# teboli/polyblur

Measured on AMD Instinct MI355X. Metric: megapixels/sec (n_iter=3, alpha=6, beta=1), higher is better.
Workload: dtype f32; 1 GPU; batch=1 3840x2160x3 fp32 per GPU, n_iter=3, method=fft (circular), full 25-tap support; mode=resident, images_per_gpu=1, height=2160, width=3840, parallelism=images sharded, no data-path collective

## Files before the change

polyblur_amd/build.py:

```python
from __future__ import annotations

import hashlib
import os
import shutil
import subprocess
import sys
from concurrent.futures import ThreadPoolExecutor

HERE = os.path.dirname(os.path.abspath(__file__))
CSRC = os.path.join(HERE, "csrc")
LIBDIR = os.path.join(HERE, "lib")
LIBNAME = "libpolyblur_hip.so"
SOURCES = ["api.hip", "comm.hip", "conv.hip", "conv_fft.hip", "conv_big.hip", "conv_wfft.hip", "conv_w128.hip", "estimate.hip", "lines_fixed.hip", "filters.hip", "nc.hip"]
EXPERIMENTAL_SOURCES = ["conv_strip.hip", "conv_xt.hip"]
ARCH = "gfx950"
FLAGS = ["-O3", "-std=c++17", "-fPIC", "--offload-arch=" + ARCH, "-Wall", "-Wno-unused-function"]


def hipcc_path() -> str:
    for cand in (os.environ.get("HIPCC"), shutil.which("hipcc"), "/opt/rocm/bin/hipcc"):
        if cand and os.path.exists(cand):
            return cand
    raise RuntimeError("hipcc not found (set HIPCC or install ROCm)")


def lib_path() -> str:
    return os.path.join(LIBDIR, LIBNAME)


def _newer(target: str, deps) -> bool:
    if not os.path.exists(target):
        return True
    t = os.path.getmtime(target)
    return any(os.path.getmtime(d) > t for d in deps)


def build(force: bool = False, verbose: bool = True, experimental: bool = False) -> str:
    os.makedirs(LIBDIR, exist_ok=True)
    hipcc = hipcc_path()
    headers = [os.path.join(CSRC, f) for f in os.listdir(CSRC) if f.endswith(".h")]
    headers.append(os.path.join(os.path.dirname(HERE), "include", "polyblur_hip.h"))
    jobs = []
    objs = []
    extra = os.environ.get("PB_EXTRA_FLAGS", "").split()
    flags = FLAGS + extra
    sources = SOURCES + (EXPERIMENTAL_SOURCES if experimental else [])
    if experimental:
        flags = flags + ["-DPB_EXPERIMENTAL"]
    flavour = hashlib.sha256(" ".join(flags + sources).encode()).hexdigest()[:10]
    objdir = os.path.join(LIBDIR, "obj" if not (extra or experimental) else "obj-" + flavour)
    os.makedirs(objdir, exist_ok=True)
    stamp = os.path.join(LIBDIR, "flavour.txt")
    relink = not os.path.exists(stamp) or open(stamp).read().strip() != flavour
    for src in sources:
        s = os.path.join(CSRC, src)
        o = os.path.join(objdir, src.replace(".hip", ".o"))
        objs.append(o)
        if force or _newer(o, [s] + headers):
            jobs.append([hipcc] + flags + ["-c", s, "-o", o])

    def run(cmd):
        if verbose:
            print(" ".join(cmd), flush=True)
        r = subprocess.run(cmd, capture_output=True, text=True)
        if r.returncode != 0:
            raise RuntimeError("hipcc failed:\n%s\n%s" % (r.stdout, r.stderr))
        if verbose and r.stderr.strip():
            print(r.stderr, file=sys.stderr)

    with ThreadPoolExecutor(max_workers=4) as ex:
        list(ex.map(run, jobs))
    out = lib_path()
    if jobs or relink or not os.path.exists(out):
        run([hipcc, "-shared", "-fPIC", "--offload-arch=" + ARCH, "-o", out] + objs + ["-ldl"])
        with open(stamp, "w") as f:
            f.write(flavour + "\n")
    return out


if __name__ == "__main__":
    print(build(force="--force" in sys.argv, experimental="--experimental" in sys.argv))
```

polyblur_amd/csrc/api.hip:

```cpp
#include <cstdlib>
#include <cstring>

#include "common.h"

int pb_grad_energy(pb_ctx *ctx, const void *gx, const void *gy, float *nM, int P, long HW, int g_dtype = PB_F32);
int pb_halo_apply(pb_ctx *ctx, const void *x, int x_dtype, int x_pitch, long x_plane, const float *y, const void *gx,
                  const void *gy, const void *ox, const float *nM, void *out, int out_dtype, int P, int H, int W,
                  int clamp01, const void *recomb_cur = nullptr, int recomb_cur_dtype = 0, const float *recomb_smooth = nullptr,
                  int g_dtype = PB_F32);
int pb_recombine(pb_ctx *ctx, const float *y, const void *cur, int cur_dtype, const float *smooth, void *out, int out_dtype,
                 long n);
int pb_bilateral5_impl(pb_ctx *ctx, const void *in, int in_dtype, void *out, int out_dtype, int P, int H, int W);
int pb_dt_filter_impl(pb_ctx *ctx, const void *in, const void *joint, int dtype, float *out, int B, int C, int H, int W,
                      float sigma_s, float sigma_r, int num_iterations);
int pb_nc_filter_impl(pb_ctx *ctx, const void *in, int dtype, float *out, int B, int C, int H, int W, float sigma_s,
                      float sigma_r, int num_iterations);
int pb_convert_from_float(pb_ctx *ctx, const float *in, void *out, int dtype, long n);
int pb_u8_layout(pb_ctx *ctx, const unsigned char *in, unsigned char *out, int B, int C, int H, int W, int to_planar);
int pb_convert_to_float(pb_ctx *ctx, const void *in, int dtype, float *out, long n);
int pb_extract_patches_impl(pb_ctx *ctx, const void *img, void *patches, int dtype, int B, int C, int H, int W, int ph, int pw,
                            int step_h, int step_w, int n_j, int pad_top, int pad_left, int first, int count);
int pb_overlap_add_impl(pb_ctx *ctx, const void *patches, void *out, int dtype, int B, int C, int H, int W, int ph, int pw,
                        int step_h, int step_w, int n_i, int n_j, int pad_top, int pad_left, const float *win_y,
                        const float *win_x);
// ... 23 lines not shown
    }
    const size_t want = (bytes + 255) & ~(size_t)255;
    if (hipMalloc(&b.p, want) != hipSuccess) {
        b.p = nullptr;
        pb_fail(ctx, PB_ERR_NOMEM, "scratch '%s': hipMalloc(%zu) failed", name, want);
        return nullptr;
    }
    b.bytes = want;
    return b.p;
}

static size_t dsize(int dtype) { return dtype == PB_F16 ? 2 : (dtype == PB_U8 ? 1 : 4); }
static int pitch4(int w) { return (w + 3) & ~3; }

static void pb_read_knobs(pb_ctx *ctx) {
    auto geti = [](const char *n, int &v) { if (const char *e = getenv(n)) v = atoi(e); };
    auto getl = [](const char *n, long &v) { if (const char *e = getenv(n)) v = atol(e); };
    if (const char *e = getenv("PB_FFT_BODY")) ctx->fft_wave = (e[0] == 'w' && e[1] == 'g') ? 0 : 1;
#ifdef PB_EXPERIMENTAL
    geti("PB_STRIP", ctx->strip_mode);
#endif
    geti("PB_EST_GRAY_ROWS", ctx->est_gray_rows); geti("PB_EST_LEAN", ctx->est_lean); geti("PB_DT_ROWS_REG", ctx->dt_rows_reg); geti("PB_DT_COLS_STRIP", ctx->dt_cols_strip); geti("PB_DT_COLS_COOP", ctx->dt_cols_coop);
    geti("PB_FFT_EXT_RADIX", ctx->fft_ext_radix); geti("PB_FFT_FIRST", ctx->fft_first); geti("PB_FFT_FIRST_ROWS", ctx->fft_first_rows); geti("PB_COLS_FIXED", ctx->cols_fixed); geti("PB_ROWS_FIXED", ctx->rows_fixed);
    geti("PB_POLY1", ctx->poly_mode);
    geti("PB_POLY_ALWAYS", ctx->poly_always); geti("PB_POLY_PADDED", ctx->poly_padded); geti("PB_TAPER_RING", ctx->taper_ring); geti("PB_ZERO_RING", ctx->zero_ring); getl("PB_ZERO_RING_MIN_PAIRS", ctx->zero_ring_min_pairs);
}

extern "C" {

int pb_version(void) { return PB_VERSION; }

void pb_default_options(pb_options *o) {
    memset(o, 0, sizeof(*o));
    o->n_iter = 1; o->c = 0.352f; o->b = 0.768f; o->alpha = 2.f; o->beta = 3.f;
    o->sigma_r = 0.8f; o->sigma_s = 2.0f; o->q = 0.f; o->n_angles = 6; o->n_interpolated_angles = 30;
    o->remove_halo = 0; o->edgetaping = 0; o->prefilter = PB_PREFILTER_NONE; o->discard_saturation = 0;
    o->boundary = PB_WRAP; o->support = PB_SUPPORT_FULL; o->force_theta_deg = -1.f; o->ker_size = PB_KSIZE;
}

int pb_create(pb_ctx **out, int device, void *stream) {
    if (!out) return PB_ERR_BADARG;
    *out = nullptr;
    int n = 0;
    if (hipGetDeviceCount(&n) != hipSuccess || n <= 0 || device < 0 || device >= n) return PB_ERR_HIP;
    if (hipSetDevice(device) != hipSuccess) return PB_ERR_HIP;
    pb_ctx *ctx = new pb_ctx();
    ctx->device = device;
    ctx->stream = static_cast<hipStream_t>(stream);
    pb_read_knobs(ctx);
    if (hipEventCreate(&ctx->ev0) != hipSuccess || hipEventCreate(&ctx->ev1) != hipSuccess ||
        hipEventCreateWithFlags(&ctx->ev_switch, hipEventDisableTiming) != hipSuccess) { delete ctx; return PB_ERR_HIP; }
    {
        if (hipStreamCreateWithFlags(&ctx->aux, hipStreamNonBlocking) != hipSuccess ||
            hipEventCreateWithFlags(&ctx->ev_fork, hipEventDisableTiming) != hipSuccess ||
            hipEventCreateWithFlags(&ctx->ev_join, hipEventDisableTiming) != hipSuccess) {
            (void)hipGetLastError();
            if (ctx->aux) (void)hipStreamDestroy(ctx->aux);
            ctx->aux = nullptr;
        }
    }
    *out = ctx;
    return PB_OK;
}

int pb_set_dense_eval(pb_ctx *ctx, int mode, int min_phases) {
    if (!ctx || (mode != PB_DENSE_STENCIL && mode != PB_DENSE_AUTO) || min_phases < 0 || min_phases > PB_MAX_PHASES + 1)
        return PB_ERR_BADARG;
    ctx->fft_min_phases = mode == PB_DENSE_STENCIL ? -1 : min_phases;
    pb_forget_hints(ctx);
    return PB_OK;
}

// ... 795 lines not shown
```

polyblur_amd/csrc/common.h:

```cpp
#pragma once
#include <hip/hip_runtime.h>
#include <hip/hip_fp16.h>

#include <cstdarg>
#include <cstdio>
#include <map>
#include <string>
#include <vector>

#include "../../include/polyblur_hip.h"


struct FftPlan {
    int n = 0;
    int nstage = 0;
    int radix[24];
    int bluestein_m = 0;
    float2 *tw = nullptr;
    float *drev = nullptr;
    float2 *chirp = nullptr;
    float2 *bfilt_rev = nullptr;
    float *dnat = nullptr;
};

// ... 66 lines not shown
    int sel_slot = 0, sel_last = 0, sel_B = 0;
    const std::vector<pb_fft_sel> *known_sel = nullptr;
    SpectraSet spectra;
    int poly_mode = 3;
    PolySpec poly_want = no_poly();
    PolySpec poly_want2 = no_poly();
    SpectraSet spectra2;
    unsigned sel2_mask = 0;
    long zero_ring_min_pairs = 4096;
    int zero_ring = 1;
    int taper_ring = 1;
    int poly_padded = 1;
    int est_lean = 1;
    int dt_cols_strip = 1;
    int dt_cols_coop = 1;
    int dt_rows_reg = 1;
    int poly_always = 1;
    int est_gray_rows = 1;
    int fft_ext_radix = 1;
    int fft_first_rows = -1;
    int fft_first = -1;
    int cols_fixed = 1;
    int rows_fixed = 1;
    int strip_mode = 0;
};

int pb_fail(pb_ctx *ctx, int code, const char *fmt, ...);

struct ProfScope {
    pb_ctx *ctx;
    int idx = -1;
    ProfScope(pb_ctx *c, int tag) : ctx(c) {
        if (!c->prof_on) return;
        ProfRec r;
        r.tag = tag;
        hipEvent_t *ev[2] = {&r.a, &r.b};
        for (auto e : ev) {
            if (!c->evpool.empty()) { *e = c->evpool.back(); c->evpool.pop_back(); }
            else if (hipEventCreate(e) != hipSuccess) return;
        }
        (void)hipEventRecord(r.a, c->stream);
        c->prof.push_back(r);
        idx = (int)c->prof.size() - 1;
    }
    ~ProfScope() {
        if (idx >= 0) (void)hipEventRecord(ctx->prof[idx].b, ctx->stream);
// ... 41 lines not shown
    void *out;       int out_kind; int out_dtype; int out_pitch; long out_plane;
    int H, W;
    int pad;
    int C;
    int P;
    const pb_blur_info *info;
    float scale, coef;
    int boundary;
    int epilogue;
    int clamp01;
    int skip_sep;
    int skip_general;
    const pb_fft_sel *fsel;
    const float *khat;
    int khat_ready;
    int strip;
    int poly;
    void *out2;  int out2_kind;  int out2_pitch;  long out2_plane;  int clamp2;
    int no_fft;
    int ring;
};

int pb_launch_conv(pb_ctx *ctx, const ConvPass &p);
int pb_launch_conv_poly(pb_ctx *ctx, const ConvPass *steps);
int pb_launch_conv_xt(pb_ctx *ctx, const ConvPass &p);
int pb_build_khat(pb_ctx *ctx, const pb_blur_info *info, int B, float **khat, pb_fft_sel **sel, bool launch);
int pb_build_khat_ring(pb_ctx *ctx, const pb_blur_info *info, int B, float **khat, pb_fft_sel **sel);
int pb_khat_buffers(pb_ctx *ctx, int B, float **khat, pb_fft_sel **sel);
int pb_khat2_buffers(pb_ctx *ctx, int B, float **khat, pb_fft_sel **sel);
inline const PolySpec &pb_spec_of_spectra(const pb_ctx *ctx, const void *khat) {
    return ctx->spectra2.built_into(khat) ? ctx->spectra2.spec() : ctx->spectra.spec();
}
int pb_cache_records(pb_ctx *ctx, const pb_blur_info *info, int B);
void pb_forget_range(pb_ctx *ctx, const void *dst, size_t bytes);
inline void pb_forget_records(pb_ctx *ctx, const void *info, int B) { pb_forget_range(ctx, info, sizeof(pb_blur_info) * (size_t)B); }
void pb_forget_hints(pb_ctx *ctx);
int pb_launch_conv_fft(pb_ctx *ctx, const ConvPass &p);
int pb_launch_conv_strip(pb_ctx *ctx, const ConvPass &p);
int pb_launch_conv_wfft(pb_ctx *ctx, const ConvPass &p);
bool pb_conv_fft_types(const ConvPass &p);
bool pb_conv_wfft_types(const ConvPass &p);
int pb_launch_conv_w128(pb_ctx *ctx, const ConvPass &p);
bool pb_conv_w128_feasible(const ConvPass &p);
bool pb_conv_wfft_feasible(const ConvPass &p, bool poly2);
bool pb_conv_w128_types(int in_dtype, int out_dtype);
bool pb_poly_three_steps_ok(pb_ctx *ctx, const ConvPass *steps);
// ... 38 lines not shown
```

polyblur_amd/csrc/conv_w128.hip:

```cpp

#include <algorithm>
#include <cstdlib>
#include <type_traits>

#include "conv_wave_common.h"

namespace {

constexpr int W_N = 128;
constexpr int W_P = 129;
constexpr size_t kW128Lds = sizeof(float2) * 64 * W_P;

static __device__ const float kC128[64] = {
    1.0f, 0.9987954497337341f, 0.9951847195625305f, 0.9891765117645264f, 0.9807852506637573f, 0.9700312614440918f,
    0.9569403529167175f, 0.9415440559387207f, 0.9238795042037964f, 0.903989315032959f, 0.8819212913513184f, 0.8577286005020142f,
    0.8314695954322815f, 0.803207516670227f, 0.7730104327201843f, 0.7409511208534241f, 0.7071067690849304f, 0.6715589761734009f,
    0.6343932747840881f, 0.5956993103027344f, 0.5555702447891235f, 0.5141027569770813f, 0.4713967442512512f, 0.4275550842285156f,
    0.3826834261417389f, 0.3368898630142212f, 0.290284663438797f, 0.24298018217086792f, 0.19509032368659973f, 0.1467304676771164f,
    0.0980171412229538f, 0.049067676067352295f, 6.123234262925839e-17f, -0.049067676067352295f, -0.0980171412229538f, -0.1467304676771164f,
    -0.19509032368659973f, -0.24298018217086792f, -0.290284663438797f, -0.3368898630142212f, -0.3826834261417389f, -0.4275550842285156f,
    -0.4713967442512512f, -0.5141027569770813f, -0.5555702447891235f, -0.5956993103027344f, -0.6343932747840881f, -0.6715589761734009f,
    -0.7071067690849304f, -0.7409511208534241f, -0.7730104327201843f, -0.803207516670227f, -0.8314695954322815f, -0.8577286005020142f,
    -0.8819212913513184f, -0.903989315032959f, -0.9238795042037964f, -0.9415440559387207f, -0.9569403529167175f, -0.9700312614440918f,
    -0.9807852506637573f, -0.9891765117645264f, -0.9951847195625305f, -0.9987954497337341f};
// ... 98 lines not shown
#define PB_WT_PASS , tr
#else
#define PB_WT(i)
#define PB_WRT(i)
#define PB_WT_ARG
#define PB_WT_PASS
#endif

struct W128Geom { int ow, oh; };
struct W128Jobs { int pairs_x, njobs, per; float inv_pairs_x; };
__device__ __forceinline__ int div_rcp128(int n, float rcp_d) { return (int)(((float)n + 0.5f) * rcp_d); }
__device__ __forceinline__ W128Jobs jobs128_of(const W128Geom &g, int hx, int hy) {
    const int Tx = W_N - 2 * hx, Ty = W_N - 2 * hy;
    const int tiles_x = div_rcp128(g.ow + Tx - 1, __builtin_amdgcn_rcpf((float)Tx)), tiles_y = div_rcp128(g.oh + Ty - 1, __builtin_amdgcn_rcpf((float)Ty));
    W128Jobs j;
    j.pairs_x = (tiles_x + 1) >> 1;
    j.njobs = j.pairs_x * tiles_y;
    j.per = (j.njobs + 7) >> 3;
    j.inv_pairs_x = __builtin_amdgcn_rcpf((float)j.pairs_x);
    return j;
}

template <typename TIn, typename TOut, bool ZERO>
__device__ __forceinline__ void w128_pair(const ConvPass &a, int plane, int ty, int pxi, int hx, int hy, float2 *Z, const float *kp PB_WT_ARG) {
    constexpr int kBoundary = ZERO ? PB_ZERO : PB_WRAP;
    const int Tx = W_N - 2 * hx, Ty = W_N - 2 * hy;
    const int w = (int)(threadIdx.x >> 6), lane = (int)(threadIdx.x & 63), c = lane & 31, h = lane >> 5;
    const bool upper = h != 0;
    const float sg = upper ? -1.f : 1.f;
    const OutRegion rg = out_region(a);
    const int oy0 = rg.y_lo + ty * Ty, wy0 = oy0 - hy;
    const int wxA = rg.x_lo + 2 * pxi * Tx - hx, wxB = wxA + Tx;
    const bool hasB = wxB + hx < rg.x_hi;
    const int x = 32 * w + c;
    const TIn *ipl = static_cast<const TIn *>(a.in) + (long)plane * a.in_plane;
    TOut *opl = static_cast<TOut *>(a.out) + (long)plane * a.out_plane;
    const int Hp = a.H + 2 * a.pad, Wp = a.W + 2 * a.pad;
    cf v[64];
    PB_WT(1);

    {
        const brsrc rin = plane_rsrc(ipl, a.in_plane);
        const int lo = a.in_kind == SRC_VIRTUAL ? a.pad : 0;
        const int pitchb = a.in_pitch * (int)sizeof(TIn);
        const bool x_inside = wxA >= lo && wxB + W_N <= Wp - lo && hasB;
        const bool y_inside = wy0 >= lo && wy0 + W_N <= Hp - lo;
        const bool inside = x_inside && y_inside;
        const bool pieces = x_inside && (y_inside || Hp >= 2 * W_N) && ((a.in_pitch | (wxA - lo)) & 3) == 0;
        if (sizeof(TIn) == 4) {
            char *zw = reinterpret_cast<char *>(Z) + w * (int)(kW128Lds / 4);
// ... 204 lines not shown
            const int row0 = 64 * h;
            const int rlo = max(hy - row0, 0), rhi = min(rmax - row0, 64);
            const unsigned baseA = okA && rlo < rhi ? (unsigned)((wy0 + row0 + rlo - oo) * opitchb + (pxA - oo) * (int)sizeof(TOut)) : kNoAccess;
            const unsigned baseB = okB && rlo < rhi ? (unsigned)((wy0 + row0 + rlo - oo) * opitchb + (pxB - oo) * (int)sizeof(TOut)) : kNoAccess;
#pragma unroll
            for (int r = 0; r < 64; ++r) {
                const bool rok = r >= rlo && r < rhi;
                cf ea = v[r], eb = v[r];
                swap_halves(ea, eb);
                const cf er = ea + eb * sg;
                const float ra = __builtin_amdgcn_fmed3f(er.x, clo, chi), rb = __builtin_amdgcn_fmed3f(er.y, clo, chi);
                BufIO<TOut>::st(ro, rok ? baseA + (unsigned)((r - rlo) * opitchb) : kNoAccess, 0, ra);
                BufIO<TOut>::st(ro, rok ? baseB + (unsigned)((r - rlo) * opitchb) : kNoAccess, 0, rb);
            }
        }
    }
    PB_WT(8);
    PB_WRT(10);
}

template <typename TIn, typename TOut, bool ZERO>
__global__ __launch_bounds__(256, 2) void conv_w128_kernel(const ConvPass a, const W128Geom g) {
    extern __shared__ __attribute__((aligned(16))) float2 Zw[];
    const int lane = threadIdx.x & 63;
#if defined(PB_EXPERIMENTAL) && defined(PB_W128_TRACE)
    unsigned long long *tr = (blockIdx.x < kTraceGroups && threadIdx.x < 64) ? g_w128_trace + (long)blockIdx.x * kTraceStamps : nullptr;
    PB_WT(0);
    PB_WRT(9);
#endif
    const int C = a.C, B = a.P / C;
    const int q = (int)(blockIdx.x & 7u);
    int rem = (int)(blockIdx.x >> 3);
    int img = 0, hx = 0, hy = 0;
    if (B == 1) {
        const PB_CONSTANT pb_fft_sel *s0 = as_constant(a.fsel);
        if (!s0->use_fft || s0->poly != 2) return;
        hx = s0->hx; hy = s0->hy;
    } else {
        auto share_of = [&](int i) -> int {
            if (i >= B) return 0;
            const pb_fft_sel s = a.fsel[i];
            if (!s.use_fft || s.poly != 2) return 0;
            return jobs128_of(g, s.hx, s.hy).per * C;
        };
        bool work = false;
        int base = 0;
        for (int c0 = 0; c0 < B; c0 += 64) {
            const int n = share_of(c0 + lane), incl = wave_scan(n, lane);
            const unsigned long long m = __ballot(base + incl > rem);
            if (m) {
                const int l = __builtin_ctzll(m);
                img = c0 + l;
                rem -= base + (__builtin_amdgcn_readlane(incl, l) - __builtin_amdgcn_readlane(n, l));
                work = true;
                break;
            }
            base += __builtin_amdgcn_readlane(incl, 63);
        }
        if (!work) return;
        img = __builtin_amdgcn_readfirstlane(img); rem = __builtin_amdgcn_readfirstlane(rem);
        hx = as_constant(a.fsel + img)->hx; hy = as_constant(a.fsel + img)->hy;
    }
    const W128Jobs j = jobs128_of(g, hx, hy);
    const int pl = __builtin_amdgcn_readfirstlane(div_rcp128(rem, __builtin_amdgcn_rcpf((float)j.per)));
    if (pl >= C) return;
    const int pair = q * j.per + (rem - pl * j.per);
    if (pair >= j.njobs) return;
    const int ty = __builtin_amdgcn_readfirstlane(div_rcp128(pair, j.inv_pairs_x)), pxi = pair - ty * j.pairs_x;
    w128_pair<TIn, TOut, ZERO>(a, img * C + pl, ty, pxi, hx, hy, Zw, a.khat + (long)img * PB_KHAT_STRIDE PB_WT_PASS);
}

template <typename TIn, typename TOut>
int launch_w128_typed(pb_ctx *ctx, const ConvPass &p, const W128Geom &g, long groups) {
    if (p.boundary == PB_ZERO)
        hipLaunchKernelGGL((conv_w128_kernel<TIn, TOut, true>), dim3((unsigned)groups), dim3(256), kW128Lds, ctx->stream, p, g);
    else
        hipLaunchKernelGGL((conv_w128_kernel<TIn, TOut, false>), dim3((unsigned)groups), dim3(256), kW128Lds, ctx->stream, p, g);
    PB_LAUNCH_CHECK();
    return PB_OK;
}

}

#if defined(PB_EXPERIMENTAL) && defined(PB_W128_TRACE)
extern "C" int pb_debug_w128_trace(unsigned long long *host) {
    int rc = (int)hipMemcpyFromSymbol(host, HIP_SYMBOL(g_w128_trace), sizeof(g_w128_trace));
    static unsigned long long zeros[kTraceGroups * kTraceStamps];
    if (!rc) rc = (int)hipMemcpyToSymbol(HIP_SYMBOL(g_w128_trace), zeros, sizeof(zeros));
    return rc;
}
#endif

// ... 11 lines not shown
    W128Geom g;
    g.oh = (p.out_kind == OUT_INTERIOR) ? p.H : p.H + 2 * p.pad;
    g.ow = (p.out_kind == OUT_INTERIOR) ? p.W : p.W + 2 * p.pad;
    long groups = 0;
    const int B = p.P / p.C;
    auto per_of = [&](int hx, int hy) -> long {
        const int tx = W_N - 2 * hx, ty = W_N - 2 * hy;
        const long nj = (long)(((g.ow + tx - 1) / tx + 1) / 2) * ((g.oh + ty - 1) / ty);
        return (nj + 7) / 8;
    };
    if (ctx->known_sel) {
        long per_sum = 0;
        for (int b = 0; b < B && b < (int)ctx->known_sel->size(); ++b) {
            const pb_fft_sel &e = (*ctx->known_sel)[(size_t)b];
            if (e.use_fft && e.poly == 2) per_sum += per_of(e.hx, e.hy);
        }
        if (!per_sum) return PB_OK;
        groups = 8L * per_sum * p.C;
    } else {
        const int hmax = (W_N - PB_POLY128_MIN_T) / 2;
        groups = 8L * per_of(hmax, hmax) * p.P;
    }
    if (groups <= 0 || groups > (1L << 23)) return pb_fail(ctx, PB_ERR_UNSUPPORTED, "conv pass: too many 128 x 128 windows");
    ProfScope prof(ctx, PB_PROF_CONV_FFT);
    switch (p.in_dtype * 3 + p.out_dtype) {
        case 0: return launch_w128_typed<float, float>(ctx, p, g, groups);
        case 1: return launch_w128_typed<float, __half>(ctx, p, g, groups);
        case 3: return launch_w128_typed<__half, float>(ctx, p, g, groups);
        case 4: return launch_w128_typed<__half, __half>(ctx, p, g, groups);
        case 2: return launch_w128_typed<float, unsigned char>(ctx, p, g, groups);
        case 5: return launch_w128_typed<__half, unsigned char>(ctx, p, g, groups);
        case 6: return launch_w128_typed<unsigned char, float>(ctx, p, g, groups);
        case 7: return launch_w128_typed<unsigned char, __half>(ctx, p, g, groups);
        case 8: return launch_w128_typed<unsigned char, unsigned char>(ctx, p, g, groups);
        default: return PB_ERR_UNSUPPORTED;
    }
}
```

polyblur_amd/csrc/conv_wave_common.h:

```cpp
#pragma once
#include "conv_fft_common.h"

namespace {

constexpr int WF_ROWS = 32;
constexpr size_t kWfLdsWave = sizeof(float2) * WF_ROWS * FT_P;

static __device__ const float kC64[64] = {
    1.0f, 0.9951847195625305f, 0.9807852506637573f, 0.9569403529167175f, 0.9238795042037964f, 0.8819212913513184f,
    0.8314695954322815f, 0.7730104327201843f, 0.7071067690849304f, 0.6343932747840881f, 0.5555702447891235f,
    0.4713967442512512f, 0.3826834261417389f, 0.290284663438797f, 0.19509032368659973f, 0.0980171412229538f, 0.0f,
    -0.0980171412229538f, -0.19509032368659973f, -0.290284663438797f, -0.3826834261417389f, -0.4713967442512512f,
    -0.5555702447891235f, -0.6343932747840881f, -0.7071067690849304f, -0.7730104327201843f, -0.8314695954322815f,
    -0.8819212913513184f, -0.9238795042037964f, -0.9569403529167175f, -0.9807852506637573f, -0.9951847195625305f, -1.0f,
    -0.9951847195625305f, -0.9807852506637573f, -0.9569403529167175f, -0.9238795042037964f, -0.8819212913513184f,
    -0.8314695954322815f, -0.7730104327201843f, -0.7071067690849304f, -0.6343932747840881f, -0.5555702447891235f,
    -0.4713967442512512f, -0.3826834261417389f, -0.290284663438797f, -0.19509032368659973f, -0.0980171412229538f, 0.0f,
    0.0980171412229538f, 0.19509032368659973f, 0.290284663438797f, 0.3826834261417389f, 0.4713967442512512f,
    0.5555702447891235f, 0.6343932747840881f, 0.7071067690849304f, 0.7730104327201843f, 0.8314695954322815f,
    0.8819212913513184f, 0.9238795042037964f, 0.9569403529167175f, 0.9807852506637573f, 0.9951847195625305f};
static __device__ const float kS64[64] = {
    0.0f, 0.0980171412229538f, 0.19509032368659973f, 0.290284663438797f, 0.3826834261417389f, 0.4713967442512512f,
    0.5555702447891235f, 0.6343932747840881f, 0.7071067690849304f, 0.7730104327201843f, 0.8314695954322815f,
    0.8819212913513184f, 0.9238795042037964f, 0.9569403529167175f, 0.9807852506637573f, 0.9951847195625305f, 1.0f,
// ... 111 lines not shown

__device__ __forceinline__ int wave_scan(int x, int lane) {
#pragma unroll
    for (int d = 1; d < 64; d <<= 1) {
        const int t = __shfl_up(x, d, 64);
        if (lane >= d) x += t;
    }
    return x;
}


#pragma clang diagnostic push
#pragma clang diagnostic ignored "-Wold-style-cast"
typedef __attribute__((address_space(3))) void lds_void;
typedef __attribute__((address_space(3))) char lds_char;
__device__ __forceinline__ lds_char *lds_ptr(void *p) { return (lds_char *)p; }
template <int IMM> __device__ __forceinline__ void dma16(brsrc r, lds_char *dst, unsigned voffset, int soffset) {
    __builtin_amdgcn_raw_ptr_buffer_load_lds(r, (lds_void *)dst, 16, (int)voffset, soffset, IMM, 0);
}
#pragma clang diagnostic pop
template <int IMM> __device__ __forceinline__ void dma4(brsrc r, lds_char *dst, unsigned voffset, int soffset) {
    __builtin_amdgcn_raw_ptr_buffer_load_lds(r, (lds_void *)dst, 4, (int)voffset, soffset, IMM, 0);
}
__device__ __forceinline__ void wait_vm0() { asm volatile("s_waitcnt vmcnt(0)" ::: "memory"); }
__device__ __forceinline__ void wait_lds0() { asm volatile("s_waitcnt lgkmcnt(0)" ::: "memory"); }
typedef float f4v __attribute__((ext_vector_type(4)));
typedef unsigned u4v __attribute__((ext_vector_type(4)));
__device__ __forceinline__ f4v ld_b128(brsrc r, unsigned voffset, int soffset) {
    return __builtin_bit_cast(f4v, __builtin_amdgcn_raw_buffer_load_b128(r, (int)voffset, soffset, 0));
}
__device__ __forceinline__ void st_b128(brsrc r, unsigned voffset, int soffset, f4v v) {
    __builtin_amdgcn_raw_buffer_store_b128(__builtin_bit_cast(u4v, v), r, (int)(voffset + (unsigned)soffset), 0, 0);
}

template <typename T> struct Piece4;
template <> struct Piece4<float> {
    typedef f4v raw;
    static __device__ __forceinline__ raw ld(brsrc r, unsigned vo, int so) { return ld_b128(r, vo, so); }
    static __device__ __forceinline__ f4v to_f(raw v) { return v; }
    static __device__ __forceinline__ void st(brsrc r, unsigned vo, int so, f4v v) { st_b128(r, vo, so, v); }
};
template <> struct Piece4<__half> {
    typedef uint2 raw;
    static __device__ __forceinline__ raw ld(brsrc r, unsigned vo, int so) {
        typedef unsigned u2v __attribute__((ext_vector_type(2)));
        const u2v t = __builtin_bit_cast(u2v, __builtin_amdgcn_raw_buffer_load_b64(r, (int)vo, so, 0));
// ... 28 lines not shown
```

polyblur_amd/csrc/conv_wfft.hip:

```cpp

#include <algorithm>
#include <cstdlib>
#include <type_traits>

#include "conv_wave_common.h"

namespace {

struct WGeom { int ow, oh; };
struct WJobs { int pairs_x, njobs, per; float inv_pairs_x; };
__device__ __forceinline__ int div_rcp(int n, float rcp_d) { return (int)(((float)n + 0.5f) * rcp_d); }
__device__ __forceinline__ WJobs jobs_of(const WGeom &g, int hx, int hy) {
    const int Tx = FT_N - 2 * hx, Ty = FT_N - 2 * hy;
    const int tiles_x = div_rcp(g.ow + Tx - 1, __builtin_amdgcn_rcpf((float)Tx)), tiles_y = div_rcp(g.oh + Ty - 1, __builtin_amdgcn_rcpf((float)Ty));
    WJobs j;
    j.pairs_x = (tiles_x + 1) >> 1;
    j.njobs = j.pairs_x * tiles_y;
    j.per = (j.njobs + 7) >> 3;
    j.inv_pairs_x = __builtin_amdgcn_rcpf((float)j.pairs_x);
    return j;
}

#ifdef PB_WF_TRACE
constexpr int kTraceWaves = 8192, kTraceStamps = 14;
// ... 1 lines not shown
#define PB_T(i) do { if (tr) { __builtin_amdgcn_sched_barrier(0); tr[i] = __builtin_readcyclecounter(); __builtin_amdgcn_sched_barrier(0); } } while (0)
#define PB_TWAIT() asm volatile("s_waitcnt vmcnt(0) lgkmcnt(0)" ::: "memory")
#define PB_TRT(i) do { if (tr) tr[i] = __builtin_amdgcn_s_memrealtime(); } while (0)
#else
#define PB_T(i)
#define PB_TWAIT()
#define PB_TRT(i)
#endif

template <int MODE, typename TIn, typename TX, typename TOut, bool ZERO>
__device__ __forceinline__ void wave_pair(const ConvPass &a, const pb_blur_info *info, int plane, int ty, int pxi, int hx, int hy,
                                          char *zb, const float *kp, unsigned long long *tr) {
    constexpr int kBoundary = ZERO ? PB_ZERO : PB_WRAP;
    constexpr bool FAST = MODE != 0, GEN = MODE == 2;
    const int Tx = FT_N - 2 * hx, Ty = FT_N - 2 * hy;
    PB_T(1);
    float2 *Z = reinterpret_cast<float2 *>(zb);
    float *Zf = reinterpret_cast<float *>(zb);
    const OutRegion rg = out_region(a);
    const int oy0 = rg.y_lo + ty * Ty;
    const int wxA = rg.x_lo + 2 * pxi * Tx - hx, wxB = wxA + Tx;
    const int wrap_r = FT_N - hy;
    const bool hasB = wxB + hx < rg.x_hi;
    const int lane = threadIdx.x & 63;
    const TIn *ipl = static_cast<const TIn *>(a.in) + (long)plane * a.in_plane;
    const TX *xpl = static_cast<const TX *>(a.x) + (long)plane * a.x_plane;
    TOut *opl = static_cast<TOut *>(a.out) + (long)plane * a.out_plane;
    const int Hp = a.H + 2 * a.pad, Wp = a.W + 2 * a.pad;
    cf v[64];

    {
        const brsrc rin = plane_rsrc(ipl, a.in_plane);
        const int lo = a.in_kind == SRC_VIRTUAL ? a.pad : 0;
        const int pitchb = a.in_pitch * (int)sizeof(TIn);
        const int wy0 = oy0 - hy;
        auto rowoff = [&](int r) -> int { return (oy0 - lo + r - (r >= wrap_r ? FT_N : 0)) * pitchb; };
        if constexpr (FAST) {
            lds_char *zl = lds_ptr(zb);
            if constexpr (sizeof(TIn) == 4) {
                const int c = lane & 31;
                const unsigned vo = (unsigned)((lane >> 5) * pitchb + ((c < 16 ? wxA : wxB - FT_N) - lo + 4 * c) * 4);
                auto request = [&](int k, int buf) {
#pragma unroll
                    for (int j = 0; j < 8; ++j) dma16<0>(rin, zl + buf * 8192 + j * 1024, vo, rowoff(8 * j + 2 * k));
                };
                const unsigned la = lds_addr(zb) + (unsigned)lane * 4u;
                auto pick = [&](int k, int buf) {
// ... 416 lines not shown

template <typename TIn, typename TX, typename TOut>
__device__ __forceinline__ bool pair_is_gen(const ConvPass &a, int pxi, int hx) {
    if (sizeof(TIn) != 4 || a.epilogue != EPI_HORNER) return false;
    const int Tx = FT_N - 2 * hx;
    const OutRegion rg = out_region(a);
    const int Wp = a.W + 2 * a.pad;
    const bool virt = a.x_kind == SRC_VIRTUAL;
    const int oo = a.out_kind == OUT_INTERIOR ? a.pad : 0, xsh = virt ? a.pad : 0, xw = virt ? a.W : Wp;
    const int oxA = rg.x_lo + 2 * pxi * Tx;
    return xw >= 4 && ((a.x_pitch | a.out_pitch | (oxA - xsh) | (oxA - oo) | (rg.x_hi - oxA) | xw) & 3) == 0;
}

__device__ __forceinline__ bool taper_is_copy(const ConvPass &a, int ty, int pxi, int hx, int hy) {
    if (a.epilogue != EPI_TAPER) return false;
    const int Tx = FT_N - 2 * hx, Ty = FT_N - 2 * hy;
    const OutRegion rg = out_region(a);
    const int Hp = a.H + 2 * a.pad, Wp = a.W + 2 * a.pad;
    const int y0 = rg.y_lo + ty * Ty, y1 = min(y0 + Ty, rg.y_hi), x0 = rg.x_lo + 2 * pxi * Tx, x1 = min(x0 + 2 * Tx, rg.x_hi);
    return y0 >= PB_KSIZE && y1 <= Hp - PB_KSIZE && x0 >= PB_KSIZE && x1 <= Wp - PB_KSIZE;
}
template <typename TX, typename TOut>
__device__ __forceinline__ void copy_pair(const ConvPass &a, int plane, int ty, int pxi, int hx, int hy) {
    const int lane = threadIdx.x & 63;
    const int Tx = FT_N - 2 * hx, Ty = FT_N - 2 * hy;
    const OutRegion rg = out_region(a);
    const int y0 = rg.y_lo + ty * Ty, y1 = min(y0 + Ty, rg.y_hi), x0 = rg.x_lo + 2 * pxi * Tx, x1 = min(x0 + 2 * Tx, rg.x_hi);
    const int xsh = a.x_kind == SRC_VIRTUAL ? a.pad : 0, oo = a.out_kind == OUT_INTERIOR ? a.pad : 0;
    const TX *xpl = static_cast<const TX *>(a.x) + (long)plane * a.x_plane;
    TOut *opl = static_cast<TOut *>(a.out) + (long)plane * a.out_plane;
    if (sizeof(TX) == 4 && sizeof(TOut) == 4 && ((a.x_pitch | a.out_pitch | (x0 - xsh) | (x0 - oo) | (x1 - x0)) & 3) == 0) {
        const int n4 = (x1 - x0) >> 2;
        const int per = 64 / n4;
        const int rl = lane / n4, pc = lane - rl * n4;
        if (rl < per) {
            for (int r = y0 + rl; r < y1; r += per) {
                const float4 v = *reinterpret_cast<const float4 *>(reinterpret_cast<const float *>(xpl) + (long)(r - xsh) * a.x_pitch + (x0 - xsh) + 4 * pc);
                *reinterpret_cast<float4 *>(reinterpret_cast<float *>(opl) + (long)(r - oo) * a.out_pitch + (x0 - oo) + 4 * pc) = v;
            }
        }
        return;
    }
    for (int r = y0; r < y1; ++r)
        for (int c = x0 + lane; c < x1; c += 64)
            pb_st(opl + (long)(r - oo) * a.out_pitch + (c - oo), pb_ld(xpl + (long)(r - xsh) * a.x_pitch + (c - xsh)));
}

__device__ __forceinline__ bool ring_live(const ConvPass &a, int ty, int pxi, int hx, int hy) {
    const int Tx = FT_N - 2 * hx, Ty = FT_N - 2 * hy;
    const OutRegion rg = out_region(a);
    const int Hp = a.H + 2 * a.pad, Wp = a.W + 2 * a.pad;
    const int y0 = rg.y_lo + ty * Ty, y1 = min(y0 + Ty, rg.y_hi), x0 = rg.x_lo + 2 * pxi * Tx, x1 = min(x0 + 2 * Tx, rg.x_hi);
    const int dy = min(y0, Hp - y1), dx = min(x0, Wp - x1);
    if (a.ring >= 4) {
        const int mt = a.ring - 4;
        return dy < 25 + 12 * mt + mt * Ty || dx < 25 + 12 * mt + 2 * mt * Tx;
    }
    const int m = 3 - a.ring;
    return dy < 24 + 12 * m + m * Ty || dx < 24 + 12 * m + 2 * m * Tx;
}

template <typename TIn, typename TX, typename TOut, bool ZERO>
__global__ __launch_bounds__(64, 2) void conv_wfft_kernel(const ConvPass a, const WGeom g) {
    extern __shared__ __attribute__((aligned(16))) char zb[];
    const int lane = threadIdx.x & 63;
    unsigned long long *tr = nullptr;
#ifdef PB_WF_TRACE
    if (blockIdx.x < kTraceWaves) tr = g_wf_trace + (long)blockIdx.x * kTraceStamps;
    PB_T(0);
    PB_TRT(12);
#endif
    const int C = a.C, B = a.P / C;
    const int q = (int)(blockIdx.x & 7u);
    int rem = (int)(blockIdx.x >> 3);
    int img = 0, hx = 0, hy = 0;
    bool fold = false;
    if (B == 1) {
        const PB_CONSTANT pb_fft_sel *s0 = as_constant(a.fsel);
        if (!s0->use_fft || s0->poly == 2 || !poly_match(a.poly, s0->poly)) return;
        hx = s0->hx; hy = s0->hy;
        fold = a.poly == 2 && s0->poly != 0;
    } else {
        auto share_of = [&](int i) -> int {
            if (i >= B) return 0;
            const pb_fft_sel s = a.fsel[i];
            if (!s.use_fft || s.poly == 2 || !poly_match(a.poly, s.poly)) return 0;
            return jobs_of(g, s.hx, s.hy).per * C;
        };
        bool work = false;
        int base = 0;
        for (int c0 = 0; c0 < B; c0 += 64) {
            const int n = share_of(c0 + lane), incl = wave_scan(n, lane);
            const unsigned long long m = __ballot(base + incl > rem);
            if (m) {
                const int l = __builtin_ctzll(m);
                img = c0 + l;
                rem -= base + (__builtin_amdgcn_readlane(incl, l) - __builtin_amdgcn_readlane(n, l));
                work = true;
                break;
            }
            base += __builtin_amdgcn_readlane(incl, 63);
        }
        if (!work) return;
        img = __builtin_amdgcn_readfirstlane(img); rem = __builtin_amdgcn_readfirstlane(rem);
        hx = as_constant(a.fsel + img)->hx; hy = as_constant(a.fsel + img)->hy;
        fold = a.poly == 2 && as_constant(a.fsel + img)->poly != 0;
    }
    const WJobs j = jobs_of(g, hx, hy);
    const int pl = __builtin_amdgcn_readfirstlane(div_rcp(rem, __builtin_amdgcn_rcpf((float)j.per)));
    if (pl >= C) return;
    const int pair = q * j.per + (rem - pl * j.per);
    if (pair >= j.njobs) return;
    const int ty = __builtin_amdgcn_readfirstlane(div_rcp(pair, j.inv_pairs_x)), pxi = pair - ty * j.pairs_x;
    const int plane = img * C + pl;
    const float *kp = a.khat + (long)img * PB_KHAT_STRIDE;
    const pb_blur_info *info = a.info + img;
    if (a.ring && !ring_live(a, ty, pxi, hx, hy)) return;
    const ConvPass af = fold_pass(a, fold);
    if (taper_is_copy(af, ty, pxi, hx, hy)) { copy_pair<TX, TOut>(af, plane, ty, pxi, hx, hy); return; }
    if (pair_is_fast<TIn, TX, TOut>(af, ty, pxi, hx, hy)) wave_pair<1, TIn, TX, TOut, ZERO>(af, info, plane, ty, pxi, hx, hy, zb, kp, tr);
    else if (pair_is_gen<TIn, TX, TOut>(af, pxi, hx)) wave_pair<2, TIn, TX, TOut, ZERO>(af, info, plane, ty, pxi, hx, hy, zb, kp, tr);
    else wave_pair<0, TIn, TX, TOut, ZERO>(af, info, plane, ty, pxi, hx, hy, zb, kp, tr);
}

bool wfft_geometry(const ConvPass &p, bool poly2, float min_area, WGeom &g, long &per_max) {
    g.oh = (p.out_kind == OUT_INTERIOR) ? p.H : p.H + 2 * p.pad;
    g.ow = (p.out_kind == OUT_INTERIOR) ? p.W : p.W + 2 * p.pad;
    per_max = 0;
    for (int hx = 4; hx <= 28; hx += 4) {
        for (int hy = 2; hy <= 30; hy += 2) {
            const int tx = FT_N - 2 * hx, ty = FT_N - 2 * hy;
            const bool three = hx <= 12 && hy <= 12;
            const bool one = poly2 && tx >= PB_POLY_MIN_TX && ty >= PB_POLY_MIN_TY && (float)(tx * ty) >= min_area;
            if (!three && !one) continue;
            const long nj = (long)(((g.ow + tx - 1) / tx + 1) / 2) * ((g.oh + ty - 1) / ty);
            if (nj > (1L << 20)) return false;
            per_max = std::max(per_max, (nj + 7) / 8);
        }
    }
    const long total = 8 * per_max * p.P;
    return total > 0 && total <= (1L << 23);
}

template <typename TIn, typename TX, typename TOut>
int launch_wfft_typed(pb_ctx *ctx, const ConvPass &p, const WGeom &g, long groups) {
// ... 36 lines not shown
    const bool poly2 = p.poly != 0 && pb_spec_of_spectra(ctx, p.khat).on >= 2;
    const float min_area = (float)PB_POLY_MIN_AREA;
    WGeom g;
    long per_max = 0;
    if (!wfft_geometry(p, poly2, min_area, g, per_max)) {
        if (poly2) return pb_fail(ctx, PB_ERR_UNSUPPORTED, "conv pass: too many windows for the tile-spectrum body");
        return PB_ERR_UNSUPPORTED;
    }
    long groups = 8L * per_max * p.P;
    if (ctx->known_sel) {
        const int B = p.P / p.C;
        long per_sum = 0, jobs = 0;
        for (int b = 0; b < B && b < (int)ctx->known_sel->size(); ++b) {
            const pb_fft_sel &e = (*ctx->known_sel)[(size_t)b];
            const bool takes = e.use_fft && e.poly != 2 && (p.poly == 2 || (e.poly != 0) == (p.poly != 0));
            if (!takes) continue;
            const int tx = FT_N - 2 * e.hx, ty = FT_N - 2 * e.hy;
            const long nj = (long)(((g.ow + tx - 1) / tx + 1) / 2) * ((g.oh + ty - 1) / ty);
            per_sum += (nj + 7) / 8; jobs += nj * p.C;
        }
        if (!jobs) return PB_OK;
        groups = 8L * per_sum * p.C;
    }
    ProfScope prof(ctx, PB_PROF_CONV_FFT);
    switch (p.in_dtype * 9 + p.x_dtype * 3 + p.out_dtype) {
        case 0: return launch_wfft_typed<float, float, float>(ctx, p, g, groups);
        case 1: return launch_wfft_typed<float, float, __half>(ctx, p, g, groups);
        case 3: return launch_wfft_typed<float, __half, float>(ctx, p, g, groups);
        case 4: return launch_wfft_typed<float, __half, __half>(ctx, p, g, groups);
        case 12: return launch_wfft_typed<__half, __half, float>(ctx, p, g, groups);
        case 13: return launch_wfft_typed<__half, __half, __half>(ctx, p, g, groups);
        case 24: return launch_wfft_typed<unsigned char, unsigned char, float>(ctx, p, g, groups);
        case 26: return launch_wfft_typed<unsigned char, unsigned char, unsigned char>(ctx, p, g, groups);
        case 6: return launch_wfft_typed<float, unsigned char, float>(ctx, p, g, groups);
        case 8: return launch_wfft_typed<float, unsigned char, unsigned char>(ctx, p, g, groups);
        case 2: return launch_wfft_typed<float, float, unsigned char>(ctx, p, g, groups);
        default: return PB_ERR_UNSUPPORTED;
    }
}
```

Before: 16980 MP/s.

## Make windowed FFT conv kernels persistent with grid-stride job loops

Converts the wfft and w128 convolution kernels from one-block-per-window launches into persistent kernels. The grid is capped at CU count times a per-CU occupancy factor, and each block loops over window jobs with a grid stride, re-resolving the image only when it crosses an image boundary. Kernel args are reloaded through scalar registers each iteration, and machine LICM is disabled for these files to limit register pressure. This trades fewer block launches and less per-block setup for a per-job barrier and possible load imbalance at the tail. It is bypassed for ring and taper passes and for the aux stream.

```diff
diff --git a/polyblur_amd/build.py b/polyblur_amd/build.py
--- a/polyblur_amd/build.py
+++ b/polyblur_amd/build.py
@@ -15,6 +15,7 @@
 EXPERIMENTAL_SOURCES = ["conv_strip.hip", "conv_xt.hip"]
 ARCH = "gfx950"
 FLAGS = ["-O3", "-std=c++17", "-fPIC", "--offload-arch=" + ARCH, "-Wall", "-Wno-unused-function"]
+SOURCE_FLAGS = {"conv_wfft.hip": ["-mllvm", "-disable-machine-licm"], "conv_w128.hip": ["-mllvm", "-disable-machine-licm"]}
 
 
 def hipcc_path() -> str:
@@ -47,7 +48,7 @@
     sources = SOURCES + (EXPERIMENTAL_SOURCES if experimental else [])
     if experimental:
         flags = flags + ["-DPB_EXPERIMENTAL"]
-    flavour = hashlib.sha256(" ".join(flags + sources).encode()).hexdigest()[:10]
+    flavour = hashlib.sha256(" ".join(flags + sources + [k + " ".join(v) for k, v in sorted(SOURCE_FLAGS.items())]).encode()).hexdigest()[:10]
     objdir = os.path.join(LIBDIR, "obj" if not (extra or experimental) else "obj-" + flavour)
     os.makedirs(objdir, exist_ok=True)
     stamp = os.path.join(LIBDIR, "flavour.txt")
@@ -57,7 +58,7 @@
         o = os.path.join(objdir, src.replace(".hip", ".o"))
         objs.append(o)
         if force or _newer(o, [s] + headers):
-            jobs.append([hipcc] + flags + ["-c", s, "-o", o])
+            jobs.append([hipcc] + flags + SOURCE_FLAGS.get(src, []) + ["-c", s, "-o", o])
 
     def run(cmd):
         if verbose:
diff --git a/polyblur_amd/csrc/api.hip b/polyblur_amd/csrc/api.hip
--- a/polyblur_amd/csrc/api.hip
+++ b/polyblur_amd/csrc/api.hip
@@ -69,7 +69,7 @@
 #endif
     geti("PB_EST_GRAY_ROWS", ctx->est_gray_rows); geti("PB_EST_LEAN", ctx->est_lean); geti("PB_DT_ROWS_REG", ctx->dt_rows_reg); geti("PB_DT_COLS_STRIP", ctx->dt_cols_strip); geti("PB_DT_COLS_COOP", ctx->dt_cols_coop);
     geti("PB_FFT_EXT_RADIX", ctx->fft_ext_radix); geti("PB_FFT_FIRST", ctx->fft_first); geti("PB_FFT_FIRST_ROWS", ctx->fft_first_rows); geti("PB_COLS_FIXED", ctx->cols_fixed); geti("PB_ROWS_FIXED", ctx->rows_fixed);
-    geti("PB_POLY1", ctx->poly_mode);
+    geti("PB_POLY1", ctx->poly_mode); geti("PB_WIN_PERSIST", ctx->win_persist);
     geti("PB_POLY_ALWAYS", ctx->poly_always); geti("PB_POLY_PADDED", ctx->poly_padded); geti("PB_TAPER_RING", ctx->taper_ring); geti("PB_ZERO_RING", ctx->zero_ring); getl("PB_ZERO_RING_MIN_PAIRS", ctx->zero_ring_min_pairs);
 }
 
@@ -95,6 +95,7 @@
     ctx->device = device;
     ctx->stream = static_cast<hipStream_t>(stream);
     pb_read_knobs(ctx);
+    if (hipDeviceGetAttribute(&ctx->cu_count, hipDeviceAttributeMultiprocessorCount, device) != hipSuccess) { (void)hipGetLastError(); ctx->cu_count = 0; }
     if (hipEventCreate(&ctx->ev0) != hipSuccess || hipEventCreate(&ctx->ev1) != hipSuccess ||
         hipEventCreateWithFlags(&ctx->ev_switch, hipEventDisableTiming) != hipSuccess) { delete ctx; return PB_ERR_HIP; }
     {
diff --git a/polyblur_amd/csrc/common.h b/polyblur_amd/csrc/common.h
--- a/polyblur_amd/csrc/common.h
+++ b/polyblur_amd/csrc/common.h
@@ -112,6 +112,8 @@
     int fft_first = -1;
     int cols_fixed = 1;
     int rows_fixed = 1;
+    int win_persist = 1;
+    int cu_count = 0;
     int strip_mode = 0;
 };
 
@@ -199,6 +201,13 @@
 };
 
 int pb_launch_conv(pb_ctx *ctx, const ConvPass &p);
+inline long pb_window_grid(const pb_ctx *ctx, const ConvPass &p, long list, int per_cu) {
+    if (ctx->win_persist <= 0) return list;
+    if (ctx->win_persist > 1) return list < ctx->win_persist ? list : (long)ctx->win_persist;
+    if (p.ring || p.epilogue == EPI_TAPER || (ctx->aux && ctx->stream == ctx->aux) || ctx->cu_count <= 0) return list;
+    const long slots = (long)ctx->cu_count * per_cu;
+    return list < slots ? list : slots;
+}
 int pb_launch_conv_poly(pb_ctx *ctx, const ConvPass *steps);
 int pb_launch_conv_xt(pb_ctx *ctx, const ConvPass &p);
 int pb_build_khat(pb_ctx *ctx, const pb_blur_info *info, int B, float **khat, pb_fft_sel **sel, bool launch);
diff --git a/polyblur_amd/csrc/conv_w128.hip b/polyblur_amd/csrc/conv_w128.hip
--- a/polyblur_amd/csrc/conv_w128.hip
+++ b/polyblur_amd/csrc/conv_w128.hip
@@ -144,10 +144,10 @@
 }
 
 template <typename TIn, typename TOut, bool ZERO>
-__device__ __forceinline__ void w128_pair(const ConvPass &a, int plane, int ty, int pxi, int hx, int hy, float2 *Z, const float *kp PB_WT_ARG) {
+__device__ __forceinline__ void w128_pair(const ConvPass &a, int w, int plane, int ty, int pxi, int hx, int hy, float2 *Z, const float *kp PB_WT_ARG) {
     constexpr int kBoundary = ZERO ? PB_ZERO : PB_WRAP;
     const int Tx = W_N - 2 * hx, Ty = W_N - 2 * hy;
-    const int w = (int)(threadIdx.x >> 6), lane = (int)(threadIdx.x & 63), c = lane & 31, h = lane >> 5;
+    const int lane = job_lane(), c = lane & 31, h = lane >> 5;
     const bool upper = h != 0;
     const float sg = upper ? -1.f : 1.f;
     const OutRegion rg = out_region(a);
@@ -398,52 +398,68 @@
 template <typename TIn, typename TOut, bool ZERO>
 __global__ __launch_bounds__(256, 2) void conv_w128_kernel(const ConvPass a, const W128Geom g) {
     extern __shared__ __attribute__((aligned(16))) float2 Zw[];
-    const int lane = threadIdx.x & 63;
-#if defined(PB_EXPERIMENTAL) && defined(PB_W128_TRACE)
-    unsigned long long *tr = (blockIdx.x < kTraceGroups && threadIdx.x < 64) ? g_w128_trace + (long)blockIdx.x * kTraceStamps : nullptr;
-    PB_WT(0);
-    PB_WRT(9);
-#endif
+    const int w = __builtin_amdgcn_readfirstlane((int)(threadIdx.x >> 6));
     const int C = a.C, B = a.P / C;
     const int q = (int)(blockIdx.x & 7u);
-    int rem = (int)(blockIdx.x >> 3);
-    int img = 0, hx = 0, hy = 0;
+    const int stride = (int)((gridDim.x + 7u - (unsigned)q) >> 3);
+    int pos = (int)(blockIdx.x >> 3);
+    int img = 0, hxi = 0, hyi = 0, lo = 0, hi = 0;
+    W128Jobs j = {0, 0, 0, 0.f};
+    float inv_per = 0.f;
     if (B == 1) {
         const PB_CONSTANT pb_fft_sel *s0 = as_constant(a.fsel);
         if (!s0->use_fft || s0->poly != 2) return;
-        hx = s0->hx; hy = s0->hy;
-    } else {
-        auto share_of = [&](int i) -> int {
-            if (i >= B) return 0;
-            const pb_fft_sel s = a.fsel[i];
-            if (!s.use_fft || s.poly != 2) return 0;
-            return jobs128_of(g, s.hx, s.hy).per * C;
-        };
-        bool work = false;
-        int base = 0;
-        for (int c0 = 0; c0 < B; c0 += 64) {
-            const int n = share_of(c0 + lane), incl = wave_scan(n, lane);
-            const unsigned long long m = __ballot(base + incl > rem);
-            if (m) {
-                const int l = __builtin_ctzll(m);
-                img = c0 + l;
-                rem -= base + (__builtin_amdgcn_readlane(incl, l) - __builtin_amdgcn_readlane(n, l));
-                work = true;
-                break;
+        hxi = s0->hx; hyi = s0->hy;
+        j = jobs128_of(g, hxi, hyi);
+        inv_per = uniform_rcp((float)j.per); j.inv_pairs_x = uniform_rcp((float)j.pairs_x);
+        hi = j.per * C;
+    }
+    for (; ; pos += stride) {
+        if (pos >= hi) {
+            if (B == 1) break;
+            auto share_of = [&](int i) -> int {
+                if (i >= B) return 0;
+                const pb_fft_sel s = a.fsel[i];
+                if (!s.use_fft || s.poly != 2) return 0;
+                return jobs128_of(g, s.hx, s.hy).per * C;
+            };
+            bool work = false;
+            int base = 0;
+            const int lane = job_lane();
+            for (int c0 = 0; c0 < B; c0 += 64) {
+                const int n = share_of(c0 + lane), incl = job_scan(n, lane);
+                const unsigned long long m = __ballot(base + incl > pos);
+                if (m) {
+                    const int l = __builtin_ctzll(m);
+                    img = c0 + l;
+                    hi = base + __builtin_amdgcn_readlane(incl, l);
+                    lo = hi - __builtin_amdgcn_readlane(n, l);
+                    work = true;
+                    break;
+                }
+                base += __builtin_amdgcn_readlane(incl, 63);
             }
-            base += __builtin_amdgcn_readlane(incl, 63);
+            if (!work) break;
+            img = __builtin_amdgcn_readfirstlane(img); lo = __builtin_amdgcn_readfirstlane(lo); hi = __builtin_amdgcn_readfirstlane(hi);
+            hxi = as_constant(a.fsel + img)->hx; hyi = as_constant(a.fsel + img)->hy;
+            j = jobs128_of(g, hxi, hyi);
+            inv_per = uniform_rcp((float)j.per); j.inv_pairs_x = uniform_rcp((float)j.pairs_x);
         }
-        if (!work) return;
-        img = __builtin_amdgcn_readfirstlane(img); rem = __builtin_amdgcn_readfirstlane(rem);
-        hx = as_constant(a.fsel + img)->hx; hy = as_constant(a.fsel + img)->hy;
-    }
-    const W128Jobs j = jobs128_of(g, hx, hy);
-    const int pl = __builtin_amdgcn_readfirstlane(div_rcp128(rem, __builtin_amdgcn_rcpf((float)j.per)));
-    if (pl >= C) return;
-    const int pair = q * j.per + (rem - pl * j.per);
-    if (pair >= j.njobs) return;
-    const int ty = __builtin_amdgcn_readfirstlane(div_rcp128(pair, j.inv_pairs_x)), pxi = pair - ty * j.pairs_x;
-    w128_pair<TIn, TOut, ZERO>(a, img * C + pl, ty, pxi, hx, hy, Zw, a.khat + (long)img * PB_KHAT_STRIDE PB_WT_PASS);
+#if defined(PB_EXPERIMENTAL) && defined(PB_W128_TRACE)
+        unsigned long long *tr = ((8 * pos + q) < kTraceGroups && w == 0) ? g_w128_trace + (long)(8 * pos + q) * kTraceStamps : nullptr;
+        PB_WT(0);
+        PB_WRT(9);
+#endif
+        const int rem = job_uniform(pos - lo);
+        const int hx = job_uniform(hxi), hy = job_uniform(hyi);
+        const int pl = __builtin_amdgcn_readfirstlane(div_rcp128(rem, inv_per));
+        const int pair = q * j.per + (rem - pl * j.per);
+        if (pair >= j.njobs) continue;
+        const int ty = __builtin_amdgcn_readfirstlane(div_rcp128(pair, j.inv_pairs_x)), pxi = pair - ty * j.pairs_x;
+        w128_pair<TIn, TOut, ZERO>(job_pass(), w, img * C + pl, ty, pxi, hx, hy, Zw, a.khat + (long)img * PB_KHAT_STRIDE PB_WT_PASS);
+        asm volatile("s_waitcnt vmcnt(0) lgkmcnt(0)" ::: "memory");
+        __syncthreads();
+    }
 }
 
 template <typename TIn, typename TOut>
@@ -501,6 +517,7 @@
         groups = 8L * per_of(hmax, hmax) * p.P;
     }
     if (groups <= 0 || groups > (1L << 23)) return pb_fail(ctx, PB_ERR_UNSUPPORTED, "conv pass: too many 128 x 128 windows");
+    groups = pb_window_grid(ctx, p, groups, 2);
     ProfScope prof(ctx, PB_PROF_CONV_FFT);
     switch (p.in_dtype * 3 + p.out_dtype) {
         case 0: return launch_w128_typed<float, float>(ctx, p, g, groups);
diff --git a/polyblur_amd/csrc/conv_wave_common.h b/polyblur_amd/csrc/conv_wave_common.h
--- a/polyblur_amd/csrc/conv_wave_common.h
+++ b/polyblur_amd/csrc/conv_wave_common.h
@@ -157,6 +157,28 @@
 template <int IMM> __device__ __forceinline__ void dma4(brsrc r, lds_char *dst, unsigned voffset, int soffset) {
     __builtin_amdgcn_raw_ptr_buffer_load_lds(r, (lds_void *)dst, 4, (int)voffset, soffset, IMM, 0);
 }
+__device__ __forceinline__ int job_lane() {
+    unsigned z = 0u;
+    asm volatile("" : "+v"(z));
+    return (int)__builtin_amdgcn_mbcnt_hi(~0u, __builtin_amdgcn_mbcnt_lo(~0u, z));
+}
+__device__ __forceinline__ int job_scan(int x, int lane) {
+#pragma unroll
+    for (int d = 1; d < 64; d <<= 1) {
+        const int t = __builtin_amdgcn_ds_bpermute(((lane - d) & 63) << 2, x);
+        if (lane >= d) x += t;
+    }
+    return x;
+}
+__device__ __forceinline__ float uniform_rcp(float d) { return __int_as_float(__builtin_amdgcn_readfirstlane(__float_as_int(__builtin_amdgcn_rcpf(d)))); }
+__device__ __forceinline__ int job_uniform(int x) { asm volatile("" : "+s"(x)); return x; }
+__device__ __forceinline__ ConvPass job_pass() {
+    auto p = __builtin_amdgcn_kernarg_segment_ptr();
+    asm volatile("" : "+s"(p));
+    ConvPass f;
+    __builtin_memcpy(&f, p, sizeof(ConvPass));
+    return f;
+}
 __device__ __forceinline__ void wait_vm0() { asm volatile("s_waitcnt vmcnt(0)" ::: "memory"); }
 __device__ __forceinline__ void wait_lds0() { asm volatile("s_waitcnt lgkmcnt(0)" ::: "memory"); }
 typedef float f4v __attribute__((ext_vector_type(4)));
diff --git a/polyblur_amd/csrc/conv_wfft.hip b/polyblur_amd/csrc/conv_wfft.hip
--- a/polyblur_amd/csrc/conv_wfft.hip
+++ b/polyblur_amd/csrc/conv_wfft.hip
@@ -47,7 +47,7 @@
     const int wxA = rg.x_lo + 2 * pxi * Tx - hx, wxB = wxA + Tx;
     const int wrap_r = FT_N - hy;
     const bool hasB = wxB + hx < rg.x_hi;
-    const int lane = threadIdx.x & 63;
+    const int lane = job_lane();
     const TIn *ipl = static_cast<const TIn *>(a.in) + (long)plane * a.in_plane;
     const TX *xpl = static_cast<const TX *>(a.x) + (long)plane * a.x_plane;
     TOut *opl = static_cast<TOut *>(a.out) + (long)plane * a.out_plane;
@@ -510,7 +510,7 @@
 }
 template <typename TX, typename TOut>
 __device__ __forceinline__ void copy_pair(const ConvPass &a, int plane, int ty, int pxi, int hx, int hy) {
-    const int lane = threadIdx.x & 63;
+    const int lane = job_lane();
     const int Tx = FT_N - 2 * hx, Ty = FT_N - 2 * hy;
     const OutRegion rg = out_region(a);
     const int y0 = rg.y_lo + ty * Ty, y1 = min(y0 + Ty, rg.y_hi), x0 = rg.x_lo + 2 * pxi * Tx, x1 = min(x0 + 2 * Tx, rg.x_hi);
@@ -551,64 +551,80 @@
 template <typename TIn, typename TX, typename TOut, bool ZERO>
 __global__ __launch_bounds__(64, 2) void conv_wfft_kernel(const ConvPass a, const WGeom g) {
     extern __shared__ __attribute__((aligned(16))) char zb[];
-    const int lane = threadIdx.x & 63;
     unsigned long long *tr = nullptr;
-#ifdef PB_WF_TRACE
-    if (blockIdx.x < kTraceWaves) tr = g_wf_trace + (long)blockIdx.x * kTraceStamps;
-    PB_T(0);
-    PB_TRT(12);
-#endif
     const int C = a.C, B = a.P / C;
     const int q = (int)(blockIdx.x & 7u);
-    int rem = (int)(blockIdx.x >> 3);
-    int img = 0, hx = 0, hy = 0;
+    const int stride = (int)((gridDim.x + 7u - (unsigned)q) >> 3);
+    int pos = (int)(blockIdx.x >> 3);
+    int img = 0, hxi = 0, hyi = 0, lo = 0, hi = 0;
     bool fold = false;
+    WJobs j = {0, 0, 0, 0.f};
+    float inv_per = 0.f;
     if (B == 1) {
         const PB_CONSTANT pb_fft_sel *s0 = as_constant(a.fsel);
         if (!s0->use_fft || s0->poly == 2 || !poly_match(a.poly, s0->poly)) return;
-        hx = s0->hx; hy = s0->hy;
+        hxi = s0->hx; hyi = s0->hy;
         fold = a.poly == 2 && s0->poly != 0;
-    } else {
-        auto share_of = [&](int i) -> int {
-            if (i >= B) return 0;
-            const pb_fft_sel s = a.fsel[i];
-            if (!s.use_fft || s.poly == 2 || !poly_match(a.poly, s.poly)) return 0;
-            return jobs_of(g, s.hx, s.hy).per * C;
-        };
-        bool work = false;
-        int base = 0;
-        for (int c0 = 0; c0 < B; c0 += 64) {
-            const int n = share_of(c0 + lane), incl = wave_scan(n, lane);
-            const unsigned long long m = __ballot(base + incl > rem);
-            if (m) {
-                const int l = __builtin_ctzll(m);
-                img = c0 + l;
-                rem -= base + (__builtin_amdgcn_readlane(incl, l) - __builtin_amdgcn_readlane(n, l));
-                work = true;
-                break;
-            }
-            base += __builtin_amdgcn_readlane(incl, 63);
-        }
-        if (!work) return;
-        img = __builtin_amdgcn_readfirstlane(img); rem = __builtin_amdgcn_readfirstlane(rem);
-        hx = as_constant(a.fsel + img)->hx; hy = as_constant(a.fsel + img)->hy;
-        fold = a.poly == 2 && as_constant(a.fsel + img)->poly != 0;
-    }
-    const WJobs j = jobs_of(g, hx, hy);
-    const int pl = __builtin_amdgcn_readfirstlane(div_rcp(rem, __builtin_amdgcn_rcpf((float)j.per)));
-    if (pl >= C) return;
-    const int pair = q * j.per + (rem - pl * j.per);
-    if (pair >= j.njobs) return;
-    const int ty = __builtin_amdgcn_readfirstlane(div_rcp(pair, j.inv_pairs_x)), pxi = pair - ty * j.pairs_x;
-    const int plane = img * C + pl;
-    const float *kp = a.khat + (long)img * PB_KHAT_STRIDE;
-    const pb_blur_info *info = a.info + img;
-    if (a.ring && !ring_live(a, ty, pxi, hx, hy)) return;
-    const ConvPass af = fold_pass(a, fold);
-    if (taper_is_copy(af, ty, pxi, hx, hy)) { copy_pair<TX, TOut>(af, plane, ty, pxi, hx, hy); return; }
-    if (pair_is_fast<TIn, TX, TOut>(af, ty, pxi, hx, hy)) wave_pair<1, TIn, TX, TOut, ZERO>(af, info, plane, ty, pxi, hx, hy, zb, kp, tr);
-    else if (pair_is_gen<TIn, TX, TOut>(af, pxi, hx)) wave_pair<2, TIn, TX, TOut, ZERO>(af, info, plane, ty, pxi, hx, hy, zb, kp, tr);
-    else wave_pair<0, TIn, TX, TOut, ZERO>(af, info, plane, ty, pxi, hx, hy, zb, kp, tr);
+        j = jobs_of(g, hxi, hyi);
+        inv_per = uniform_rcp((float)j.per); j.inv_pairs_x = uniform_rcp((float)j.pairs_x);
+        hi = j.per * C;
+    }
+    for (; ; pos += stride) {
+        if (pos >= hi) {
+            if (B == 1) break;
+            auto share_of = [&](int i) -> int {
+                if (i >= B) return 0;
+                const pb_fft_sel s = a.fsel[i];
+                if (!s.use_fft || s.poly == 2 || !poly_match(a.poly, s.poly)) return 0;
+                return jobs_of(g, s.hx, s.hy).per * C;
+            };
+            bool work = false;
+            int base = 0;
+            const int lane = job_lane();
+            for (int c0 = 0; c0 < B; c0 += 64) {
+                const int n = share_of(c0 + lane), incl = job_scan(n, lane);
+                const unsigned long long m = __ballot(base + incl > pos);
+                if (m) {
+                    const int l = __builtin_ctzll(m);
+                    img = c0 + l;
+                    hi = base + __builtin_amdgcn_readlane(incl, l);
+                    lo = hi - __builtin_amdgcn_readlane(n, l);
+                    work = true;
+                    break;
+                }
+                base += __builtin_amdgcn_readlane(incl, 63);
+            }
+            if (!work) break;
+            img = __builtin_amdgcn_readfirstlane(img); lo = __builtin_amdgcn_readfirstlane(lo); hi = __builtin_amdgcn_readfirstlane(hi);
+            hxi = as_constant(a.fsel + img)->hx; hyi = as_constant(a.fsel + img)->hy;
+            fold = a.poly == 2 && as_constant(a.fsel + img)->poly != 0;
+            j = jobs_of(g, hxi, hyi);
+            inv_per = uniform_rcp((float)j.per); j.inv_pairs_x = uniform_rcp((float)j.pairs_x);
+        }
+#ifdef PB_WF_TRACE
+        tr = (8 * pos + q) < kTraceWaves ? g_wf_trace + (long)(8 * pos + q) * kTraceStamps : nullptr;
+        PB_T(0);
+        PB_TRT(12);
+#endif
+        const int rem = job_uniform(pos - lo);
+        const int hx = job_uniform(hxi), hy = job_uniform(hyi);
+        const int pl = __builtin_amdgcn_readfirstlane(div_rcp(rem, inv_per));
+        const int pair = q * j.per + (rem - pl * j.per);
+        if (pair >= j.njobs) continue;
+        const int ty = __builtin_amdgcn_readfirstlane(div_rcp(pair, j.inv_pairs_x)), pxi = pair - ty * j.pairs_x;
+        const int plane = img * C + pl;
+        const float *kp = a.khat + (long)img * PB_KHAT_STRIDE;
+        const pb_blur_info *info = a.info + img;
+        const ConvPass aj = job_pass();
+        if (aj.ring && !ring_live(aj, ty, pxi, hx, hy)) continue;
+        const ConvPass af = fold_pass(aj, fold);
+        if (taper_is_copy(af, ty, pxi, hx, hy)) copy_pair<TX, TOut>(af, plane, ty, pxi, hx, hy);
+        else if (pair_is_fast<TIn, TX, TOut>(af, ty, pxi, hx, hy)) wave_pair<1, TIn, TX, TOut, ZERO>(af, info, plane, ty, pxi, hx, hy, zb, kp, tr);
+        else if (pair_is_gen<TIn, TX, TOut>(af, pxi, hx)) wave_pair<2, TIn, TX, TOut, ZERO>(af, info, plane, ty, pxi, hx, hy, zb, kp, tr);
+        else wave_pair<0, TIn, TX, TOut, ZERO>(af, info, plane, ty, pxi, hx, hy, zb, kp, tr);
+        asm volatile("s_waitcnt vmcnt(0) lgkmcnt(0)" ::: "memory");
+        wave_lds_fence();
+    }
 }
 
 bool wfft_geometry(const ConvPass &p, bool poly2, float min_area, WGeom &g, long &per_max) {
@@ -691,6 +707,7 @@
         if (!jobs) return PB_OK;
         groups = 8L * per_sum * p.C;
     }
+    groups = pb_window_grid(ctx, p, groups, 8);
     ProfScope prof(ctx, PB_PROF_CONV_FFT);
     switch (p.in_dtype * 9 + p.x_dtype * 3 + p.out_dtype) {
         case 0: return launch_wfft_typed<float, float, float>(ctx, p, g, groups);
```

Result: slower. 15030 MP/s (-11.5%).
